# Gabrielcb/DaliID

Hardware: AMD Instinct MI355X
Metric: images/sec (train step) (higher is better)
Workload: dtype bf16; 1 GPU; configs[1]: ResNet-50 ReID bf16 256x128, PK batch 16x16=256 per GPU, center+proxy heads, Adam, EMA; global_batch=256, per_gpu_batch=256, parallelism=dp1

## Files before the change

### daliid_amd/csrc/conv.hip

```cpp
#include "gemm_tile.h"
#include "kernels.h"
#include <cstdlib>
#include <type_traits>
#include <vector>
#include <string>
#include <cstdio>

namespace dali {

__device__ __forceinline__ void decode_pixel(const GatherGeom& g, int p, int& n, int& ho, int& wo) {
    if (g.lhw >= 0 && g.lw >= 0) {
        n = p >> g.lhw;
        const int rem = p & ((1 << g.lhw) - 1);
        ho = rem >> g.lw;
        wo = rem & ((1 << g.lw) - 1);
    } else {
        const int hw = g.Hout * g.Wout;
        n = p / hw;
        const int rem = p - n * hw;
        ho = rem / g.Wout;
        wo = rem - ho * g.Wout;
    }
}

// ... 1295 lines not shown
                const bf16x8_t fb = *reinterpret_cast<const bf16x8_t*>(patch + (boff[j] ^ (uint32_t)(h << 5)));
#pragma unroll
                for (int i = 0; i < FM; ++i) acc[i][j] = __builtin_amdgcn_mfma_f32_16x16x32_bf16(fa[i], fb, acc[i][j], 0, 0, 0);
            }
        }
        asm volatile("s_waitcnt lgkmcnt(0)" ::: "memory");
        __builtin_amdgcn_s_barrier();
    }
    conv_epilogue_g<TM, TN, FM, FN, 4, NT, (EPI == 3 || EPI == 5) ? EPI : 2>(a, acc, 0, tn, smem, 0, wn);
}

}
#include "fused1x1.h"
namespace dali {

__device__ __forceinline__ int wg_swz(int row) { return (row & 3) | (((row >> 3) & 1) << 2); }

typedef short s16x4_t __attribute__((ext_vector_type(4)));

__device__ __forceinline__ bf16x8_t tr_frag(const uint16_t* tile, int chunk32, int lane) {
    const int g = lane >> 4, q = (lane & 15) >> 2, p = lane & 3;
    const int row0 = 8 * g + q, row1 = row0 + 4;
    const int off0 = row0 * 128 + ((chunk32 ^ wg_swz(row0)) << 4) + 4 * p;
    const int off1 = row1 * 128 + ((chunk32 ^ wg_swz(row1)) << 4) + 4 * p;
    typedef __attribute__((address_space(3))) s16x4_t* lds_ptr_t;
    const s16x4_t a = __builtin_amdgcn_ds_read_tr16_b64_v4i16((lds_ptr_t)(tile + off0));
    const s16x4_t b = __builtin_amdgcn_ds_read_tr16_b64_v4i16((lds_ptr_t)(tile + off1));
    typedef short s16x8_t __attribute__((ext_vector_type(8)));
    const s16x8_t v = {a[0], a[1], a[2], a[3], b[0], b[1], b[2], b[3]};
    return __builtin_bit_cast(bf16x8_t, v);
}

struct TrPair { s16x4_t lo, hi; };
__device__ __forceinline__ s16x4_t ds_read_tr_raw(const uint16_t* p) {
    typedef __attribute__((address_space(3))) const uint16_t* lds_cptr_t;
    const uint32_t addr = (uint32_t)(uintptr_t)(lds_cptr_t)p;
    s16x4_t v;
    asm volatile("ds_read_b64_tr_b16 %0, %1" : "=v"(v) : "v"(addr));
    return v;
}
__device__ __forceinline__ TrPair tr_frag_raw(const uint16_t* tile, int chunk32, int lane) {
    const int g = lane >> 4, q = (lane & 15) >> 2, p = lane & 3;
    const int row0 = 8 * g + q, row1 = row0 + 4;
    const int off0 = row0 * 128 + ((chunk32 ^ wg_swz(row0)) << 4) + 4 * p;
    const int off1 = row1 * 128 + ((chunk32 ^ wg_swz(row1)) << 4) + 4 * p;
    return TrPair{ds_read_tr_raw(tile + off0), ds_read_tr_raw(tile + off1)};
// ... 2 lines not shown
    typedef short s16x8_t __attribute__((ext_vector_type(8)));
    const s16x8_t v = {t.lo[0], t.lo[1], t.lo[2], t.lo[3], t.hi[0], t.hi[1], t.hi[2], t.hi[3]};
    return __builtin_bit_cast(bf16x8_t, v);
}
template <int N>
__device__ __forceinline__ void tr_settle(TrPair& a, TrPair& b, TrPair& c, TrPair& d) {
    static_assert(N == 0 || N == 8 || N == 10 || N == 16 || N == 18, "lgkmcnt immediates used by the callers");
    if constexpr (N == 0) asm volatile("s_waitcnt lgkmcnt(0)" : "+v"(a.lo), "+v"(a.hi), "+v"(b.lo), "+v"(b.hi), "+v"(c.lo), "+v"(c.hi), "+v"(d.lo), "+v"(d.hi));
    else if constexpr (N == 8) asm volatile("s_waitcnt lgkmcnt(8)" : "+v"(a.lo), "+v"(a.hi), "+v"(b.lo), "+v"(b.hi), "+v"(c.lo), "+v"(c.hi), "+v"(d.lo), "+v"(d.hi));
    else if constexpr (N == 10) asm volatile("s_waitcnt lgkmcnt(10)" : "+v"(a.lo), "+v"(a.hi), "+v"(b.lo), "+v"(b.hi), "+v"(c.lo), "+v"(c.hi), "+v"(d.lo), "+v"(d.hi));
    else if constexpr (N == 16) asm volatile("s_waitcnt lgkmcnt(15)" : "+v"(a.lo), "+v"(a.hi), "+v"(b.lo), "+v"(b.hi), "+v"(c.lo), "+v"(c.hi), "+v"(d.lo), "+v"(d.hi));
    else asm volatile("s_waitcnt lgkmcnt(15)" : "+v"(a.lo), "+v"(a.hi), "+v"(b.lo), "+v"(b.hi), "+v"(c.lo), "+v"(c.hi), "+v"(d.lo), "+v"(d.hi));
}

__device__ __forceinline__ void tr_settle_all(TrPair& a) { asm volatile("s_waitcnt lgkmcnt(0)" : "+v"(a.lo), "+v"(a.hi)); }

template <int FM, int FN>
__device__ __forceinline__ void store_slab_tiles(float* slab, const f32x4_t (&acc)[FM][FN], int m_first, int n_first, int Cm, int Ntot, int lane) {
    const int mr = m_first + (lane >> 4) * 4, nc = n_first + (lane & 15);
    if (m_first + 16 * FM <= Cm && n_first + 16 * FN <= Ntot) {
        float* row = slab + (size_t)mr * Ntot + nc;
#pragma unroll
        for (int i = 0; i < FM; ++i)
#pragma unroll
            for (int rr = 0; rr < 4; ++rr) {
                float* p = row + (size_t)(i * 16 + rr) * Ntot;
#pragma unroll
                for (int j = 0; j < FN; ++j) p[j * 16] = acc[i][j][rr];
            }
        return;
    }
#pragma unroll
    for (int i = 0; i < FM; ++i)
#pragma unroll
        for (int j = 0; j < FN; ++j) {
            const int n = nc + j * 16;
#pragma unroll
            for (int rr = 0; rr < 4; ++rr) {
                const int m = mr + i * 16 + rr;
                if (m < Cm && n < Ntot) slab[(size_t)m * Ntot + n] = acc[i][j][rr];
            }
        }
}

template <bool IN_BN>
__global__ __launch_bounds__(256) void igemm_wgrad_kernel(WGradArgs a, int tiles_m, int tiles_n) {
    constexpr int TILE = 32 * 128;
    __shared__ __attribute__((aligned(16))) uint16_t smem[2 * 2 * TILE];
    const int tid = threadIdx.x, lane = tid & 63, wave = tid >> 6;
    const int wm = wave >> 1, wn = wave & 1;
    const int tiles = tiles_m * tiles_n;
    const int tile = blockIdx.x % tiles, ks = blockIdx.x / tiles;
    const int tm = tile / tiles_n, tn = tile - tm * tiles_n;
    const int m0 = tm * 128, n0 = tn * 128;
    const GatherGeom g = a.g;

    const int c16 = tid & 15;
    const int am = m0 + c16 * 8;
// ... 1565 lines not shown
```

### daliid_amd/csrc/kernels.h

```cpp
#pragma once
#include "common.h"

namespace dali {

struct GatherGeom {
    int Hout, Wout;
    int Hin, Win;
    int Ck;
    int R, S, stride, pad;
    int mode;
    long long img_pitch;
    int row_pitch, pix_pitch;
    int lw, lhw;
    int sub, oph, opw, Hfull, Wfull;
    int r0, rstep, nr, s0, sstep, ns;
    int class_grid;
};

struct IGemmArgs {
    const uint16_t* W;
    const uint16_t* X;
    uint16_t* O;
    const uint16_t* Res;
    const uint8_t* res_mask;
// ... 31 lines not shown
    float* colsum;
};


struct TransposeJob { const uint16_t* w; uint16_t* wt; int Co, T, Ci, first_block; };
int launch_weight_transpose_batched(hipStream_t st, const TransposeJob* jobs, int n);

struct BnBwdSide { const uint16_t* raw; const float* mean; const float* invstd; const float* scale; const float* shift; };

int launch_igemm_conv(hipStream_t st, const IGemmArgs& a);
int gemm_profile_begin(hipStream_t st, int cls, double flops, const char* what);
void gemm_profile_end(hipStream_t st, int slot);
int igemm_conv_stat_tiles(int Cm, int P, int K);
bool conv_cat_act_supported(int Cm, int c1, int c2, int P, int parts = 1);
void wgrad_plan(int Cm, int Ntot, int P, int target_blocks, int* splits, int* pix_per_split, size_t* ws_bytes, int taps = 1, int halo_w = 0);
int launch_igemm_wgrad(hipStream_t st, const WGradArgs& a, float* out, int accumulate, float* colsum_out = nullptr, int colsum_rows = 0);
int launch_splitk_reduce2(hipStream_t st, const float* partial, float* out, size_t elems, int splits, int accumulate,
                          const float* partial2, float* out2, size_t elems2, int splits2);
bool wgrad_colsum_supported(int Cm, int Ntot, int taps, int P);
int launch_splitk_reduce(hipStream_t st, const float* partial, float* out, size_t elems, int splits, int accumulate);

int launch_linear_fwd(hipStream_t st, const uint16_t* x, const uint16_t* w, const float* bias, int act, const uint16_t* residual, uint16_t* y,
                      uint16_t* pre, const uint16_t* dact_pre, int rows, int K, int N, const float* row_scale = nullptr);
int launch_linear_wgrad(hipStream_t st, const uint16_t* x, const uint16_t* dy, float* dw, int rows, int K, int N, float* slab,
                        float* dbias = nullptr, float* cs_partial = nullptr, bool* bias_done = nullptr);
size_t linear_wgrad_colsum_floats(int rows, int K, int N);
int wgrad_colsum_rows(int Cm, int Ntot, int taps, int P, int splits);
size_t linear_wgrad_slab_bytes(int rows, int K, int N);

int launch_bnlin_stats(hipStream_t st, const uint16_t* W, const uint16_t* Wt, const float* gram, const float* m2, int C, int w, double count, const float* gamma,
// ... 6 lines not shown

constexpr int REDUCE_SMAX = 64;
inline size_t reduce_scratch_bytes(int C, int NV) { return (size_t)REDUCE_SMAX * C * NV * sizeof(double); }
int launch_bn_finalize(hipStream_t st, const float* partial, int tiles, int C, double count, const float* gamma, const float* beta,
                       float* rm, float* rv, float momentum, float eps, float* scale, float* shift, float* mean, float* invstd,
                       double* scratch);
int launch_bn_eval_coeffs(hipStream_t st, const float* gamma, const float* beta, const float* rm, const float* rv, float eps, int C,
                          float* scale, float* shift);
struct BnEvalJob { const float *gamma, *beta, *rm, *rv; float *scale, *shift; int C; };
struct BnEvalJobs { static constexpr int MAX = 56; BnEvalJob job[MAX]; };
int launch_bn_eval_coeffs_batched(hipStream_t st, const BnEvalJob* jobs, int n, float eps);
int launch_fold_cat_weights(hipStream_t st, const float* w3, const float* wd, const float* s3, const float* sd, const float* h3, const float* hd, int C, int w,
                            int cin, int parts, uint16_t* wcat, float* shcat);
int launch_bn_act(hipStream_t st, const uint16_t* raw, const float* scale, const float* shift, const uint16_t* idn, const uint16_t* raw2,
                  const float* scale2, const float* shift2, int relu, size_t elems, int C, uint16_t* y, uint8_t* mask_out);
int bn_bwd_blocks(int P, int C, int* rows_per_block);
size_t bn_bwd_partial_floats(int P, int C, bool dual);
int launch_bn_bwd(hipStream_t st, const uint16_t* g, const uint16_t* ymask, const uint8_t* ybits, const BnBwdSide& a, const BnBwdSide* b, int relu, int P, int C,
                  float* partial, float* coef_a, float* coef_b, float* dgamma_a, float* dbeta_a, float* dgamma_b, float* dbeta_b,
                  uint16_t* draw_a, uint16_t* draw_b, uint16_t* dz_out, double* scratch);
int launch_stem_pack_image(hipStream_t st, const float* img, int N, int H, int W, uint16_t* out);
int launch_stem_pack_weight(hipStream_t st, const float* w, int Cout, uint16_t* out);
bool stem_fused_supported(int N, int H, int W, int C);
bool stem_train_supported(int N, int H, int W, int C);
int stem_train_tiles(int N, int H);
int launch_stem_conv_stats(hipStream_t st, const uint16_t* ximg, const uint16_t* w_packed, int N, int H, int W, uint16_t* raw, float* stats);
int launch_stem_conv_bn_pool(hipStream_t st, const uint16_t* ximg, const uint16_t* w_packed, const float* scale, const float* shift, int N, int H, int W,
                             uint16_t* out);
int launch_stem_unpack_wgrad(hipStream_t st, const float* padded, int Cout, float* dw);
int launch_maxpool_bn_fwd(hipStream_t st, const uint16_t* raw, const float* scale, const float* shift, int N, int H, int W, int C,
// ... 35 lines not shown
```

### daliid_amd/csrc/nnops.hip

```cpp
#include "kernels.h"
#include "reduce_finish.h"

namespace dali {

__device__ __forceinline__ void unpack8(const uint4& v, float (&f)[8]) {
    f[0] = bf16_bits_to_f32(v.x & 0xffffu); f[1] = bf16_bits_to_f32(v.x >> 16);
    f[2] = bf16_bits_to_f32(v.y & 0xffffu); f[3] = bf16_bits_to_f32(v.y >> 16);
    f[4] = bf16_bits_to_f32(v.z & 0xffffu); f[5] = bf16_bits_to_f32(v.z >> 16);
    f[6] = bf16_bits_to_f32(v.w & 0xffffu); f[7] = bf16_bits_to_f32(v.w >> 16);
}
__device__ __forceinline__ uint4 pack8(const float (&f)[8]) {
    return make_uint4(pack_bf16x2(f[0], f[1]), pack_bf16x2(f[2], f[3]), pack_bf16x2(f[4], f[5]), pack_bf16x2(f[6], f[7]));
}
__device__ __forceinline__ void load8f(const float* __restrict__ p, float (&f)[8]) {
    const float4 a = *reinterpret_cast<const float4*>(p), b = *reinterpret_cast<const float4*>(p + 4);
    f[0] = a.x; f[1] = a.y; f[2] = a.z; f[3] = a.w; f[4] = b.x; f[5] = b.y; f[6] = b.z; f[7] = b.w;
}

struct FinBnFwd {
    double count;
    const float *gamma, *beta;
    float *running_mean, *running_var;
    float momentum, eps;
    float *scale, *shift, *mean_out, *invstd_out;
// ... 273 lines not shown
__global__ void stem_pack_weight_kernel(const float* __restrict__ w, int Cout, uint16_t* __restrict__ out) {
    const int i = blockIdx.x * blockDim.x + threadIdx.x;
    if (i >= Cout * 224) return;
    const int c = i & 3, s = (i >> 2) & 7, r = (i >> 5) % 7, o = i / 224;
    float v = 0.f;
    if (c < 3 && s < 7) v = w[((o * 7 + r) * 7 + s) * 3 + c];
    out[i] = f32_to_bf16_bits(v);
}
__global__ void stem_unpack_wgrad_kernel(const float* __restrict__ padded, int Cout, float* __restrict__ dw) {
    const int i = blockIdx.x * blockDim.x + threadIdx.x;
    if (i >= Cout * 147) return;
    const int c = i % 3, s = (i / 3) % 7, r = (i / 21) % 7, o = i / 147;
    dw[i] = padded[((o * 7 + r) * 8 + s) * 4 + c];
}

__global__ __launch_bounds__(256) void maxpool_bn_fwd_kernel(const uint16_t* __restrict__ raw, const float* __restrict__ scale,
                                                              const float* __restrict__ shift, int N, int H, int W, int C,
                                                              int Ho, int Wo, uint16_t* __restrict__ out, uint8_t* __restrict__ arg) {
    const int cpr = C >> 3;
    const size_t total = (size_t)N * Ho * Wo * cpr;
    for (size_t i = (size_t)blockIdx.x * 256 + threadIdx.x; i < total; i += (size_t)gridDim.x * 256) {
        const int cc = (int)(i % cpr) * 8;
        const size_t pix = i / cpr;
        const int wo = (int)(pix % Wo), ho = (int)((pix / Wo) % Ho), n = (int)(pix / ((size_t)Wo * Ho));
        float sc[8], sh[8], best[8];
        int bi[8];
        load8f(scale + cc, sc); load8f(shift + cc, sh);
#pragma unroll
        for (int t = 0; t < 8; ++t) { best[t] = -__builtin_inff(); bi[t] = 0; }
        uint4 q[9];
        bool ok[9];
#pragma unroll
        for (int r = 0; r < 3; ++r) {
            const int h = ho * 2 - 1 + r, hc = h < 0 ? 0 : (h >= H ? H - 1 : h);
#pragma unroll
            for (int s2 = 0; s2 < 3; ++s2) {
                const int w = wo * 2 - 1 + s2, wc = w < 0 ? 0 : (w >= W ? W - 1 : w);
                ok[r * 3 + s2] = h >= 0 && h < H && w >= 0 && w < W;
                q[r * 3 + s2] = *reinterpret_cast<const uint4*>(raw + (((size_t)n * H + hc) * W + wc) * C + cc);
            }
        }
#pragma unroll
        for (int k = 0; k < 9; ++k) {
            float v[8];
            unpack8(q[k], v);
#pragma unroll
            for (int t = 0; t < 8; ++t) {
                const float z = v[t] * sc[t] + sh[t];
                if (ok[k] && z > best[t]) { best[t] = z; bi[t] = k; }
            }
        }
        *reinterpret_cast<uint4*>(out + pix * C + cc) = pack8(best);
        uint32_t lo = 0, hi = 0;
#pragma unroll
        for (int t = 0; t < 4; ++t) { lo |= (uint32_t)bi[t] << (8 * t); hi |= (uint32_t)bi[t + 4] << (8 * t); }
        *reinterpret_cast<uint2*>(arg + pix * C + cc) = make_uint2(lo, hi);
    }
}

__device__ __forceinline__ void maxpool_gather_dz(const uint16_t* __restrict__ dp, const uint8_t* __restrict__ arg, int n, int h, int w,
                                                  int cc, int C, int Ho, int Wo, float (&dz)[8]) {
    const int ho0 = h >> 1, wo0 = w >> 1;
    const int rh[2] = {1 + (h & 1), 0}, rw[2] = {1 + (w & 1), 0};
    const bool vh[2] = {ho0 < Ho, (h & 1) && ho0 + 1 < Ho}, vw[2] = {wo0 < Wo, (w & 1) && wo0 + 1 < Wo};
    uint4 gq[4];
    uint2 aq[4];
#pragma unroll
    for (int k = 0; k < 4; ++k) {
        const int a = k >> 1, b = k & 1;
        const int ho = min(ho0 + a, Ho - 1), wo = min(wo0 + b, Wo - 1);
        const size_t o = (((size_t)n * Ho + ho) * Wo + wo) * C + cc;
        aq[k] = *reinterpret_cast<const uint2*>(arg + o);
// ... 437 lines not shown
    return DALI_OK;
}
int launch_fold_cat_weights(hipStream_t st, const float* w3, const float* wd, const float* s3, const float* sd, const float* h3, const float* hd, int C, int w,
                            int cin, int parts, uint16_t* wcat, float* shcat) {
    const size_t n = (size_t)C * parts * (w + cin);
    hipLaunchKernelGGL(fold_cat_weights_kernel, dim3(grid_for(n, 1024)), dim3(256), 0, st, w3, wd, s3, sd, h3, hd, C, w, cin, parts, wcat, shcat);
    DALI_LAUNCH_CHECK();
    return DALI_OK;
}
int launch_bn_act(hipStream_t st, const uint16_t* raw, const float* scale, const float* shift, const uint16_t* idn, const uint16_t* raw2,
                  const float* scale2, const float* shift2, int relu, size_t elems, int C, uint16_t* y, uint8_t* mask_out) {
    const size_t chunks = elems / 8;
    hipLaunchKernelGGL(bn_act_kernel, dim3(grid_for(chunks)), dim3(256), 0, st, raw, scale, shift, idn, raw2, scale2, shift2, relu, chunks, C, y, mask_out);
    DALI_LAUNCH_CHECK();
    return DALI_OK;
}
int bn_bwd_blocks(int P, int C, int* rows_per_block) {
    const int rif = 256 / (C / 8);
    int blocks = (P + rif * 8 - 1) / (rif * 8);
    if (blocks > 1024) blocks = 1024;
    if (blocks < 1) blocks = 1;
    int rpb = (P + blocks - 1) / blocks;
    rpb = (rpb + rif - 1) / rif * rif;
    blocks = (P + rpb - 1) / rpb;
    *rows_per_block = rpb;
    return blocks;
}
int launch_bn_bwd(hipStream_t st, const uint16_t* g, const uint16_t* ymask, const uint8_t* ybits, const BnBwdSide& a, const BnBwdSide* b, int relu, int P, int C,
                  float* partial, float* coef_a, float* coef_b, float* dgamma_a, float* dbeta_a, float* dgamma_b, float* dbeta_b,
                  uint16_t* draw_a, uint16_t* draw_b, uint16_t* dz_out, double* scratch) {
// ... 183 lines not shown
    float* coef_b = reinterpret_cast<float*>(ws + align_up(pf * 4, 256) + align_up((size_t)C * 12, 256));
    double* scratch = reinterpret_cast<double*>(ws + align_up(pf * 4, 256) + 2 * align_up((size_t)C * 12, 256));
    BnBwdSide a{raw_a, mean_a, invstd_a, scale_a, shift_a};
    BnBwdSide b{raw_b, mean_b, invstd_b, scale_b, nullptr};
    return launch_bn_bwd((hipStream_t)stream, g, ymask, ybits, a, dual ? &b : nullptr, relu, (int)pixels, C, partial, coef_a, coef_b, dgamma_a, dbeta_a,
                         dgamma_b, dbeta_b, draw_a, draw_b, dz_out, scratch);
}

extern "C" int dali_maxpool_bn_fwd(dali_ctx* ctx, void* stream, const uint16_t* raw, const float* scale, const float* shift, int n, int h,
                                   int w, int C, uint16_t* out, uint8_t* arg) {
    DALI_REQUIRE(ctx && raw && scale && shift && out && arg, "dali_maxpool_bn_fwd: null argument");
    DALI_REQUIRE(C % 8 == 0 && n > 0 && h > 0 && w > 0, "dali_maxpool_bn_fwd: bad shape");
    return launch_maxpool_bn_fwd((hipStream_t)stream, raw, scale, shift, n, h, w, C, out, arg);
}

extern "C" int dali_maxpool_bn_bwd(dali_ctx* ctx, void* stream, const uint16_t* dpool, const uint8_t* arg, const uint16_t* raw,
                                   const float* mean, const float* invstd, const float* scale, int n, int h, int w, int C,
                                   float* dgamma, float* dbeta, uint16_t* draw) {
    DALI_REQUIRE(ctx && dpool && arg && raw && mean && invstd && scale && dgamma && dbeta && draw, "dali_maxpool_bn_bwd: null argument");
    DALI_REQUIRE(C % 8 == 0 && C <= 2048, "dali_maxpool_bn_bwd: C must be a multiple of 8, <= 2048");
    const size_t pf = bn_bwd_partial_floats(n * h * w, C, false);
    const size_t need = align_up(pf * 4, 256) + align_up((size_t)C * 12, 256) + reduce_scratch_bytes(C, 2);
    char* ws = static_cast<char*>(workspace(ctx, need));
    if (!ws) return DALI_ERR_NOMEM;
    return launch_maxpool_bn_bwd((hipStream_t)stream, dpool, arg, raw, mean, invstd, scale, n, h, w, C, reinterpret_cast<float*>(ws),
                                 reinterpret_cast<float*>(ws + align_up(pf * 4, 256)), dgamma, dbeta, draw,
                                 reinterpret_cast<double*>(ws + align_up(pf * 4, 256) + align_up((size_t)C * 12, 256)));
}

extern "C" int dali_head_pool_fwd(dali_ctx* ctx, void* stream, const uint16_t* x, int n, int hw, int C, int mode, float* f, int16_t* arg) {
// ... 24 lines not shown
```

### daliid_amd/csrc/resnet_plan.hip

```cpp
#include "kernels.h"
#include <cstdio>
#include <cstring>
#include <new>
#include <string>
#include <vector>

using namespace dali;

namespace {

struct TensorInfo { std::string name; int64_t offset, numel; int shape[4]; int ndim; };

struct Conv {
    int cin, cout, r, s, stride, pad, hin, win, hout, wout;
    int64_t w_off;
    uint16_t* w_bf16;
    uint16_t* wt_bf16;
};
struct Bn {
    int C;
    int64_t g_off, b_off;
    int64_t rm_off, rv_off;
    float *scale, *shift, *mean, *invstd, *coef;
};
// ... 389 lines not shown
}

extern "C" int dali_resnet_forward(dali_resnet* net, void* stream, const float* images, int training, float* emb) {
    DALI_REQUIRE(net && net->P && images && emb, "dali_resnet_forward: null argument or net not bound");
    hipStream_t st = (hipStream_t)stream;
    const bool tr = training != 0;
    net->fwd_training = tr;
    int rc;
    if (!tr) {
        std::vector<BnEvalJob> jobs;
        auto add = [&](Bn& b) { jobs.push_back(BnEvalJob{net->P + b.g_off, net->P + b.b_off, net->B + b.rm_off, net->B + b.rv_off, b.scale, b.shift, b.C}); };
        add(net->stem_bn);
        for (auto& b : net->blocks) { add(b.b1); add(b.b2); add(b.b3); if (b.has_ds) add(b.bd); }
        if ((rc = launch_bn_eval_coeffs_batched(st, jobs.data(), (int)jobs.size(), 1e-5f))) return rc;
    }
    if ((rc = launch_stem_pack_image(st, images, net->N, net->H, net->W, net->ximg))) return rc;
    if (!tr && stem_fused_supported(net->N, net->H, net->W, net->stem.cout)) {
        if ((rc = launch_stem_conv_bn_pool(st, net->ximg, net->w_stem, net->stem_bn.scale, net->stem_bn.shift, net->N, net->H, net->W, net->pool0))) return rc;
    } else {
    if (tr && stem_train_supported(net->N, net->H, net->W, net->stem.cout)) {
        if ((rc = launch_stem_conv_stats(st, net->ximg, net->w_stem, net->N, net->H, net->W, net->raw0, net->stat_partial))) return rc;
        if ((rc = bn_train(net, st, net->stem_bn, stem_train_tiles(net->N, net->H), (double)net->N * net->stem_h * net->stem_w))) return rc;
    } else {
        IGemmArgs a{};
        a.W = net->w_stem; a.X = net->ximg; a.O = net->raw0; a.Res = nullptr; a.in_scale = nullptr; a.in_shift = nullptr; a.in_relu = 0;
        a.stats = tr ? net->stat_partial : nullptr;
        a.Cm = net->stem.cout; a.P = net->N * net->stem_h * net->stem_w;
        a.g = stem_geom(net);
        if ((rc = launch_igemm_conv(st, a))) return rc;
        if (tr && (rc = bn_train(net, st, net->stem_bn, igemm_conv_stat_tiles(a.Cm, a.P, 224), (double)a.P))) return rc;
    }
    if ((rc = launch_maxpool_bn_fwd(st, net->raw0, net->stem_bn.scale, net->stem_bn.shift, net->N, net->stem_h, net->stem_w, net->stem.cout,
                                    net->pool0, net->pool_arg))) return rc;
    }
    const uint16_t* x = net->pool0;
    for (auto& b : net->blocks) {
        b.x = const_cast<uint16_t*>(x);
        const size_t e1 = (size_t)net->N * b.hin * b.win * b.width, e2 = (size_t)net->N * b.hout * b.wout * b.width;
        if (!tr) {
            if ((rc = conv_bn_relu_eval(net, st, b.c1, b.b1, x, b.a1))) return rc;
            if ((rc = conv_bn_relu_eval(net, st, b.c2, b.b2, b.a1, b.a2))) return rc;
        } else {
            if ((rc = conv_bn_fwd(net, st, b.c1, b.b1, x, nullptr, b.raw1, tr))) return rc;
            if ((rc = launch_bn_act(st, b.raw1, b.b1.scale, b.b1.shift, nullptr, nullptr, nullptr, nullptr, 1, e1, b.width, b.a1, nullptr))) return rc;
            if ((rc = conv_bn_fwd(net, st, b.c2, b.b2, b.a1, nullptr, b.raw2, tr))) return rc;
            if ((rc = launch_bn_act(st, b.raw2, b.b2.scale, b.b2.shift, nullptr, nullptr, nullptr, nullptr, 1, e2, b.width, b.a2, nullptr))) return rc;
        }
        const int Pout = net->N * b.hout * b.wout;
        if (tr) {
            const Conv sq = square_conv(b.c3);
            WGradArgs wa{};
            wa.dY = b.a2; wa.X = b.a2; wa.partial = net->wgrad_slab; wa.Cm = b.width; wa.P = Pout; wa.Ntot = b.width;
            wa.g = conv_geom(sq, 0);
            size_t wsb;
            wgrad_plan(wa.Cm, wa.Ntot, wa.P, 512, &wa.splits, &wa.pix_per_split, &wsb, 1, 0);
            const bool fused_cs = wgrad_colsum_supported(wa.Cm, wa.Ntot, 1, wa.P);
            if (fused_cs) wa.colsum = net->cs_partial;
            if ((rc = launch_igemm_wgrad(st, wa, b.gram, 0, fused_cs ? b.m2 : nullptr, fused_cs ? wgrad_colsum_rows(wa.Cm, wa.Ntot, 1, wa.P, wa.splits) : 0))) return rc;
            if (!fused_cs && (rc = launch_colsum(st, b.a2, Pout, b.width, b.m2, net->cs_partial, net->red_scratch))) return rc;
            if ((rc = launch_bnlin_stats(st, b.c3.w_bf16, b.c3.wt_bf16, b.gram, b.m2, b.cout, b.width, (double)Pout, net->P + b.b3.g_off, net->P + b.b3.b_off,
                                         net->B + b.b3.rm_off, net->B + b.b3.rv_off, 0.1f, 1e-5f, b.ut, b.dot, b.b3.scale, b.b3.shift, b.b3.mean,
                                         b.b3.invstd))) return rc;
        }
        if (!tr && b.cat_eval) {
            if ((rc = launch_fold_cat_weights(st, net->P + b.c3.w_off, net->P + b.cd.w_off, b.b3.scale, b.bd.scale, b.b3.shift, b.bd.shift, b.cout, b.width,
                                              b.cin, 2, b.wcat, b.shcat))) return rc;
            IGemmArgs ca{};
            ca.W = b.wcat; ca.X = b.a2; ca.X2 = x; ca.Ck1 = b.width; ca.x_rep = 2; ca.O = b.y; ca.out_shift = b.shcat; ca.out_relu = 1;
            ca.Cm = b.cout; ca.P = Pout;
            Conv cat = b.c3;
            cat.cin = 2 * (b.width + b.cin);
            ca.g = conv_geom(cat, 0);
            if ((rc = launch_igemm_conv(st, ca))) return rc;
            x = b.y;
            continue;
        }
        IGemmArgs a{};
        a.W = b.c3.w_bf16; a.X = b.a2; a.O = b.y; a.Res = x; a.out_scale = b.b3.scale; a.out_shift = b.b3.shift; a.out_relu = 1;
        if (b.has_ds) {
            if ((rc = conv_bn_fwd(net, st, b.cd, b.bd, x, nullptr, b.rawd, tr))) return rc;
            a.Res = b.rawd; a.res_scale = b.bd.scale; a.bias = b.bd.shift;
            if (b.lin_ds && tr) {
                Conv sq = b.cd;
                sq.cout = b.cd.cin;
                WGradArgs wa{};
                wa.dY = x; wa.X = x; wa.partial = net->wgrad_slab; wa.Cm = b.cin; wa.P = Pout; wa.Ntot = b.cin;
                wa.g = conv_geom(sq, 0);
                size_t wsb;
                wgrad_plan(wa.Cm, wa.Ntot, wa.P, 512, &wa.splits, &wa.pix_per_split, &wsb, 1, 0);
                const bool fused_cs = wgrad_colsum_supported(wa.Cm, wa.Ntot, 1, wa.P);
                if (fused_cs) wa.colsum = net->cs_partial;
                if ((rc = launch_igemm_wgrad(st, wa, b.gram_d, 0, fused_cs ? b.m2_d : nullptr, fused_cs ? wgrad_colsum_rows(wa.Cm, wa.Ntot, 1, wa.P, wa.splits) : 0))) return rc;
                if (!fused_cs && (rc = launch_colsum(st, x, Pout, b.cin, b.m2_d, net->cs_partial, net->red_scratch))) return rc;
                if ((rc = launch_bnlin_ut(st, b.cd.w_bf16, b.gram_d, b.cout, b.cin, b.ut_d))) return rc;
            }
        }
        a.bits_out = tr ? b.ybits : nullptr;
        a.Cm = b.cout; a.P = Pout; a.g = conv_geom(b.c3, 0);
        if ((rc = launch_igemm_conv(st, a))) return rc;
        x = b.y;
    }
    if ((rc = launch_head_pool_fwd(st, x, net->N, net->head_hw, net->feat_dim, net->feature_mode, net->feat, net->head_arg))) return rc;
    return launch_bn1d_fwd(st, net->feat, net->N, net->feat_dim, net->P + net->neck.g_off, net->P + net->neck.b_off, net->B + net->neck.rm_off,
                           net->B + net->neck.rv_off, tr ? 1 : 0, 0.1f, 1e-5f, emb, net->neck_mean, net->neck_invstd);
}

static int block_backward(dali_resnet* net, hipStream_t st, Block& b, const uint8_t* prev_bits) {
    int rc;
    uint16_t* dz = net->cur_dy;
    const int Pout = net->N * b.hout * b.wout, Pin = net->N * b.hin * b.win;
// ... 174 lines not shown
```

### include/daliid_debug.h

```cpp
#ifndef DALIID_DEBUG_H
#define DALIID_DEBUG_H

#ifdef __cplusplus
extern "C" {
#endif

int dali_debug_reload_env(void);

int dali_debug_set_conv_stamps(void* dev_ptr);

int dali_debug_wgrad_splits(int Cm, int Ntot, int P, int taps, int halo_w);

int dali_debug_splitk_reduce(void* stream, const float* partial, float* out, long long elems, int splits, int accumulate);

struct dali_resnet;
int dali_debug_resnet_backward_block(struct dali_resnet* net, void* stream, const float* d_emb, int block);

#ifdef __cplusplus
}
#endif
#endif
```

Measured before the change: 17400 images/s.

## Fuse BN-activation and maxpool with Gram/colsum computation for linearized BN stats

Adds two fused kernels. One applies BN+ReLU to the conv2 output while also computing the activation's Gram matrix and column sums via MFMA. The other does the stem maxpool+BN and the Gram matrix for the first downsample block. These replace the separate bn_act pass plus a re-read of the activation by the wgrad Gram kernel, saving a full activation read and a kernel launch per block. The cost is more complex kernels whose occupancy and split planning may differ from the tuned wgrad path. The fused path falls back when shapes are not covered.

```diff
diff --git a/daliid_amd/csrc/conv.hip b/daliid_amd/csrc/conv.hip
--- a/daliid_amd/csrc/conv.hip
+++ b/daliid_amd/csrc/conv.hip
@@ -1,5 +1,6 @@
 #include "gemm_tile.h"
 #include "kernels.h"
+#include "wgrad_frag.h"
 #include <cstdlib>
 #include <type_traits>
 #include <vector>
@@ -1333,22 +1334,6 @@
 #include "fused1x1.h"
 namespace dali {
 
-__device__ __forceinline__ int wg_swz(int row) { return (row & 3) | (((row >> 3) & 1) << 2); }
-
-typedef short s16x4_t __attribute__((ext_vector_type(4)));
-
-__device__ __forceinline__ bf16x8_t tr_frag(const uint16_t* tile, int chunk32, int lane) {
-    const int g = lane >> 4, q = (lane & 15) >> 2, p = lane & 3;
-    const int row0 = 8 * g + q, row1 = row0 + 4;
-    const int off0 = row0 * 128 + ((chunk32 ^ wg_swz(row0)) << 4) + 4 * p;
-    const int off1 = row1 * 128 + ((chunk32 ^ wg_swz(row1)) << 4) + 4 * p;
-    typedef __attribute__((address_space(3))) s16x4_t* lds_ptr_t;
-    const s16x4_t a = __builtin_amdgcn_ds_read_tr16_b64_v4i16((lds_ptr_t)(tile + off0));
-    const s16x4_t b = __builtin_amdgcn_ds_read_tr16_b64_v4i16((lds_ptr_t)(tile + off1));
-    typedef short s16x8_t __attribute__((ext_vector_type(8)));
-    const s16x8_t v = {a[0], a[1], a[2], a[3], b[0], b[1], b[2], b[3]};
-    return __builtin_bit_cast(bf16x8_t, v);
-}
 
 struct TrPair { s16x4_t lo, hi; };
 __device__ __forceinline__ s16x4_t ds_read_tr_raw(const uint16_t* p) {
@@ -1381,34 +1366,6 @@
 }
 
 __device__ __forceinline__ void tr_settle_all(TrPair& a) { asm volatile("s_waitcnt lgkmcnt(0)" : "+v"(a.lo), "+v"(a.hi)); }
-
-template <int FM, int FN>
-__device__ __forceinline__ void store_slab_tiles(float* slab, const f32x4_t (&acc)[FM][FN], int m_first, int n_first, int Cm, int Ntot, int lane) {
-    const int mr = m_first + (lane >> 4) * 4, nc = n_first + (lane & 15);
-    if (m_first + 16 * FM <= Cm && n_first + 16 * FN <= Ntot) {
-        float* row = slab + (size_t)mr * Ntot + nc;
-#pragma unroll
-        for (int i = 0; i < FM; ++i)
-#pragma unroll
-            for (int rr = 0; rr < 4; ++rr) {
-                float* p = row + (size_t)(i * 16 + rr) * Ntot;
-#pragma unroll
-                for (int j = 0; j < FN; ++j) p[j * 16] = acc[i][j][rr];
-            }
-        return;
-    }
-#pragma unroll
-    for (int i = 0; i < FM; ++i)
-#pragma unroll
-        for (int j = 0; j < FN; ++j) {
-            const int n = nc + j * 16;
-#pragma unroll
-            for (int rr = 0; rr < 4; ++rr) {
-                const int m = mr + i * 16 + rr;
-                if (m < Cm && n < Ntot) slab[(size_t)m * Ntot + n] = acc[i][j][rr];
-            }
-        }
-}
 
 template <bool IN_BN>
 __global__ __launch_bounds__(256) void igemm_wgrad_kernel(WGradArgs a, int tiles_m, int tiles_n) {
diff --git a/daliid_amd/csrc/kernels.h b/daliid_amd/csrc/kernels.h
--- a/daliid_amd/csrc/kernels.h
+++ b/daliid_amd/csrc/kernels.h
@@ -69,6 +69,7 @@
 int igemm_conv_stat_tiles(int Cm, int P, int K);
 bool conv_cat_act_supported(int Cm, int c1, int c2, int P, int parts = 1);
 void wgrad_plan(int Cm, int Ntot, int P, int target_blocks, int* splits, int* pix_per_split, size_t* ws_bytes, int taps = 1, int halo_w = 0);
+int wgrad_pick_cfg(int Cm, int Ntot, int taps, int P, int halo_w);
 int launch_igemm_wgrad(hipStream_t st, const WGradArgs& a, float* out, int accumulate, float* colsum_out = nullptr, int colsum_rows = 0);
 int launch_splitk_reduce2(hipStream_t st, const float* partial, float* out, size_t elems, int splits, int accumulate,
                           const float* partial2, float* out2, size_t elems2, int splits2);
@@ -105,6 +106,12 @@
                             int cin, int parts, uint16_t* wcat, float* shcat);
 int launch_bn_act(hipStream_t st, const uint16_t* raw, const float* scale, const float* shift, const uint16_t* idn, const uint16_t* raw2,
                   const float* scale2, const float* shift2, int relu, size_t elems, int C, uint16_t* y, uint8_t* mask_out);
+bool bn_act_gram_supported(int P, int w);
+int launch_bn_act_gram(hipStream_t st, const uint16_t* raw, const float* scale, const float* shift, int P, int w, uint16_t* y, float* slab,
+                       float* cs_slab, float* gram, float* m2);
+bool maxpool_bn_gram_supported(int N, int H, int W, int C);
+int launch_maxpool_bn_gram(hipStream_t st, const uint16_t* raw, const float* scale, const float* shift, int N, int H, int W, int C, uint16_t* out,
+                           uint8_t* arg, float* slab, float* cs_slab, float* gram, float* m2);
 int bn_bwd_blocks(int P, int C, int* rows_per_block);
 size_t bn_bwd_partial_floats(int P, int C, bool dual);
 int launch_bn_bwd(hipStream_t st, const uint16_t* g, const uint16_t* ymask, const uint8_t* ybits, const BnBwdSide& a, const BnBwdSide* b, int relu, int P, int C,
diff --git a/daliid_amd/csrc/nnops.hip b/daliid_amd/csrc/nnops.hip
--- a/daliid_amd/csrc/nnops.hip
+++ b/daliid_amd/csrc/nnops.hip
@@ -1,5 +1,7 @@
 #include "kernels.h"
 #include "reduce_finish.h"
+#include "wgrad_frag.h"
+#include <cstdio>
 
 namespace dali {
 
@@ -311,6 +313,29 @@
     dw[i] = padded[((o * 7 + r) * 8 + s) * 4 + c];
 }
 
+__device__ __forceinline__ void maxpool_bn_taps(const uint4 (&q)[9], const bool (&ok)[9], const float (&sc)[8], const float (&sh)[8], uint4& out,
+                                                uint2& arg) {
+    float best[8];
+    int bi[8];
+#pragma unroll
+    for (int t = 0; t < 8; ++t) { best[t] = -__builtin_inff(); bi[t] = 0; }
+#pragma unroll
+    for (int k = 0; k < 9; ++k) {
+        float v[8];
+        unpack8(q[k], v);
+#pragma unroll
+        for (int t = 0; t < 8; ++t) {
+            const float z = v[t] * sc[t] + sh[t];
+            if (ok[k] && z > best[t]) { best[t] = z; bi[t] = k; }
+        }
+    }
+    out = pack8(best);
+    uint32_t lo = 0, hi = 0;
+#pragma unroll
+    for (int t = 0; t < 4; ++t) { lo |= (uint32_t)bi[t] << (8 * t); hi |= (uint32_t)bi[t + 4] << (8 * t); }
+    arg = make_uint2(lo, hi);
+}
+
 __global__ __launch_bounds__(256) void maxpool_bn_fwd_kernel(const uint16_t* __restrict__ raw, const float* __restrict__ scale,
                                                               const float* __restrict__ shift, int N, int H, int W, int C,
                                                               int Ho, int Wo, uint16_t* __restrict__ out, uint8_t* __restrict__ arg) {
@@ -320,11 +345,8 @@
         const int cc = (int)(i % cpr) * 8;
         const size_t pix = i / cpr;
         const int wo = (int)(pix % Wo), ho = (int)((pix / Wo) % Ho), n = (int)(pix / ((size_t)Wo * Ho));
-        float sc[8], sh[8], best[8];
-        int bi[8];
+        float sc[8], sh[8];
         load8f(scale + cc, sc); load8f(shift + cc, sh);
-#pragma unroll
-        for (int t = 0; t < 8; ++t) { best[t] = -__builtin_inff(); bi[t] = 0; }
         uint4 q[9];
         bool ok[9];
 #pragma unroll
@@ -337,22 +359,192 @@
                 q[r * 3 + s2] = *reinterpret_cast<const uint4*>(raw + (((size_t)n * H + hc) * W + wc) * C + cc);
             }
         }
-#pragma unroll
-        for (int k = 0; k < 9; ++k) {
-            float v[8];
-            unpack8(q[k], v);
-#pragma unroll
-            for (int t = 0; t < 8; ++t) {
-                const float z = v[t] * sc[t] + sh[t];
-                if (ok[k] && z > best[t]) { best[t] = z; bi[t] = k; }
+        uint4 o;
+        uint2 oa;
+        maxpool_bn_taps(q, ok, sc, sh, o, oa);
+        *reinterpret_cast<uint4*>(out + pix * C + cc) = o;
+        *reinterpret_cast<uint2*>(arg + pix * C + cc) = oa;
+    }
+}
+
+struct BnGramArgs {
+    const uint16_t* raw;
+    const float *scale, *shift;
+    uint16_t* out;
+    uint8_t* arg;
+    float *partial, *colsum;
+    int pps;
+    int H, Ho;
+};
+
+template <int W>
+struct GramTiles {
+    static constexpr int FM = W == 64 ? 1 : 4, FN = 4;
+    int mf0, nf0;
+    bool do_cs;
+    f32x4_t acc[FM][FN], cs[FM];
+    __device__ explicit GramTiles(int wave) {
+        mf0 = W == 64 ? wave : (wave >> 1) * 4;
+        nf0 = W == 64 ? 0 : (wave & 1) * 4;
+        do_cs = W == 64 || (wave & 1) == 0;
+#pragma unroll
+        for (int i = 0; i < FM; ++i) {
+            cs[i] = f32x4_t{0.f, 0.f, 0.f, 0.f};
+#pragma unroll
+            for (int j = 0; j < FN; ++j) acc[i][j] = f32x4_t{0.f, 0.f, 0.f, 0.f};
+        }
+    }
+    __device__ void step(const uint16_t* img, int lane) {
+        typedef short ones_vec_t __attribute__((ext_vector_type(8)));
+        const bf16x8_t ones = __builtin_bit_cast(bf16x8_t, ones_vec_t{0x3F80, 0x3F80, 0x3F80, 0x3F80, 0x3F80, 0x3F80, 0x3F80, 0x3F80});
+        bf16x8_t fa[FM];
+#pragma unroll
+        for (int i = 0; i < FM; ++i) fa[i] = tr_frag(img, mf0 + i, lane);
+#pragma unroll
+        for (int j = 0; j < FN; ++j) {
+            const bf16x8_t fb = tr_frag(img, nf0 + j, lane);
+#pragma unroll
+            for (int i = 0; i < FM; ++i) acc[i][j] = __builtin_amdgcn_mfma_f32_16x16x32_bf16(fa[i], fb, acc[i][j], 0, 0, 0);
+        }
+        if (do_cs) {
+#pragma unroll
+            for (int i = 0; i < FM; ++i) cs[i] = __builtin_amdgcn_mfma_f32_16x16x32_bf16(fa[i], ones, cs[i], 0, 0, 0);
+        }
+    }
+    __device__ void store(const BnGramArgs& a, int ks, int lane) const {
+        store_slab_tiles<FM, FN>(a.partial + (size_t)ks * W * W, acc, 16 * mf0, 16 * nf0, W, W, lane);
+        if (do_cs && (lane & 15) == 0) {
+#pragma unroll
+            for (int i = 0; i < FM; ++i)
+#pragma unroll
+                for (int rr = 0; rr < 4; ++rr) a.colsum[(size_t)ks * W + 16 * (mf0 + i) + (lane >> 4) * 4 + rr] = cs[i][rr];
+        }
+    }
+};
+
+template <int W, int U>
+__global__ __launch_bounds__(256, 2) void bn_act_gram_kernel(BnGramArgs a) {
+    static_assert(W == 64 || W == 128, "widths of the plan");
+    constexpr int CPR = W / 8, RSTEP = 256 / CPR;
+    constexpr int CPT = CPR / 8;
+    constexpr int NB = U * CPT;
+    __shared__ __attribute__((aligned(16))) uint16_t smem[U * 32 * 128];
+    const int tid = threadIdx.x, lane = tid & 63;
+    const int wave = __builtin_amdgcn_readfirstlane(tid >> 6);
+    const int ks = blockIdx.x;
+    const int c16 = tid % CPR, row0 = tid / CPR;
+    float sc[8], sh[8];
+    load8f(a.scale + c16 * 8, sc); load8f(a.shift + c16 * 8, sh);
+    auto load = [&](int ph, uint4 (&q)[NB]) {
+#pragma unroll
+        for (int u = 0; u < U; ++u)
+#pragma unroll
+            for (int c = 0; c < CPT; ++c) {
+                const size_t pix = (size_t)ks * a.pps + (ph * U + u) * 32 + row0 + c * RSTEP;
+                q[u * CPT + c] = *reinterpret_cast<const uint4*>(a.raw + pix * W + c16 * 8);
             }
-        }
-        *reinterpret_cast<uint4*>(out + pix * C + cc) = pack8(best);
-        uint32_t lo = 0, hi = 0;
-#pragma unroll
-        for (int t = 0; t < 4; ++t) { lo |= (uint32_t)bi[t] << (8 * t); hi |= (uint32_t)bi[t + 4] << (8 * t); }
-        *reinterpret_cast<uint2*>(arg + pix * C + cc) = make_uint2(lo, hi);
-    }
+    };
+    GramTiles<W> gt(wave);
+    const int nph = a.pps / (32 * U);
+    uint4 cur[NB], nxt[NB];
+    load(0, cur);
+    for (int ph = 0; ph < nph; ++ph) {
+        if (ph + 1 < nph) load(ph + 1, nxt);
+#pragma unroll
+        for (int u = 0; u < U; ++u)
+#pragma unroll
+            for (int c = 0; c < CPT; ++c) {
+                const int row = row0 + c * RSTEP;
+                const size_t pix = (size_t)ks * a.pps + (ph * U + u) * 32 + row;
+                float v[8];
+                unpack8(cur[u * CPT + c], v);
+#pragma unroll
+                for (int t = 0; t < 8; ++t) v[t] = v[t] * sc[t] + sh[t];
+#pragma unroll
+                for (int t = 0; t < 8; ++t) v[t] = fmaxf(v[t], 0.f);
+                const uint4 o = pack8(v);
+                *reinterpret_cast<uint4*>(a.out + pix * W + c16 * 8) = o;
+                *reinterpret_cast<uint4*>(smem + u * 32 * 128 + wg_img_off(row, c16)) = o;
+            }
+        __syncthreads();
+#pragma unroll
+        for (int u = 0; u < U; ++u) gt.step(smem + u * 32 * 128, lane);
+        __syncthreads();
+#pragma unroll
+        for (int i = 0; i < NB; ++i) cur[i] = nxt[i];
+    }
+    gt.store(a, ks, lane);
+}
+
+typedef uint32_t u32x4_t __attribute__((ext_vector_type(4)));
+template <int U>
+__global__ __launch_bounds__(256, 2) void maxpool_bn_gram_kernel(BnGramArgs a) {
+    constexpr int C = 64, WIN = 64, WO = 32, ROWS = 2 * U + 1, RB = WIN * C;
+    constexpr int NB = ROWS * 2;
+    __shared__ __attribute__((aligned(16))) uint16_t stage[ROWS * RB];
+    __shared__ __attribute__((aligned(16))) uint16_t smem[U * 32 * 128];
+    const int tid = threadIdx.x, lane = tid & 63;
+    const int wave = __builtin_amdgcn_readfirstlane(tid >> 6);
+    const int ks = blockIdx.x;
+    const int c16 = tid & 7, wo = tid >> 3;
+    float sc[8], sh[8];
+    load8f(a.scale + c16 * 8, sc); load8f(a.shift + c16 * 8, sh);
+    auto rows_of = [&](int ph, int& n, int& ho0) __attribute__((always_inline)) {
+        const int t = (ks * a.pps) / WO + ph * U;
+        n = t / a.Ho; ho0 = t - n * a.Ho;
+    };
+    auto load = [&](int ph, u32x4_t (&q)[NB]) __attribute__((always_inline)) {
+        int n, ho0;
+        rows_of(ph, n, ho0);
+#pragma unroll
+        for (int j = 0; j < ROWS; ++j) {
+            const int h = 2 * ho0 - 1 + j, hc = h < 0 ? 0 : (h >= a.H ? a.H - 1 : h);
+#pragma unroll
+            for (int c = 0; c < 2; ++c)
+                q[j * 2 + c] = *reinterpret_cast<const u32x4_t*>(a.raw + ((size_t)n * a.H + hc) * RB + (tid + 256 * c) * 8);
+        }
+    };
+    GramTiles<C> gt(wave);
+    const int nph = a.pps / (32 * U);
+    u32x4_t rg[NB];
+    load(0, rg);
+    for (int ph = 0; ph < nph; ++ph) {
+#pragma unroll
+        for (int j = 0; j < ROWS; ++j)
+#pragma unroll
+            for (int c = 0; c < 2; ++c) *reinterpret_cast<u32x4_t*>(stage + j * RB + (tid + 256 * c) * 8) = rg[j * 2 + c];
+        __syncthreads();
+        if (ph + 1 < nph) load(ph + 1, rg);
+        int n, ho0;
+        rows_of(ph, n, ho0);
+#pragma unroll
+        for (int u = 0; u < U; ++u) {
+            const int ho = ho0 + u;
+            uint4 q[9];
+            bool ok[9];
+#pragma unroll
+            for (int r = 0; r < 3; ++r) {
+                const int h = ho * 2 - 1 + r;
+#pragma unroll
+                for (int s2 = 0; s2 < 3; ++s2) {
+                    const int w = wo * 2 - 1 + s2, wc = w < 0 ? 0 : (w >= WIN ? WIN - 1 : w);
+                    ok[r * 3 + s2] = h >= 0 && h < a.H && w >= 0 && w < WIN;
+                    q[r * 3 + s2] = *reinterpret_cast<const uint4*>(stage + (2 * u + r) * RB + wc * C + c16 * 8);
+                }
+            }
+            uint4 o;
+            uint2 oa;
+            maxpool_bn_taps(q, ok, sc, sh, o, oa);
+            const size_t pix = ((size_t)n * a.Ho + ho) * WO + wo;
+            *reinterpret_cast<uint4*>(a.out + pix * C + c16 * 8) = o;
+            *reinterpret_cast<uint2*>(a.arg + pix * C + c16 * 8) = oa;
+            *reinterpret_cast<uint4*>(smem + u * 32 * 128 + wg_img_off(wo, c16)) = o;
+        }
+        __syncthreads();
+#pragma unroll
+        for (int u = 0; u < U; ++u) gt.step(smem + u * 32 * 128, lane);
+    }
+    gt.store(a, ks, lane);
 }
 
 __device__ __forceinline__ void maxpool_gather_dz(const uint16_t* __restrict__ dp, const uint8_t* __restrict__ arg, int n, int h, int w,
@@ -820,6 +1012,51 @@
     hipLaunchKernelGGL(bn_act_kernel, dim3(grid_for(chunks)), dim3(256), 0, st, raw, scale, shift, idn, raw2, scale2, shift2, relu, chunks, C, y, mask_out);
     DALI_LAUNCH_CHECK();
     return DALI_OK;
+}
+
+constexpr int BNG_U64 = 8, BNG_U128 = 4, BNG_U_POOL = 2;
+static int bn_gram_splits(int P, int w, int u, int* pps) {
+    if (!(w == 64 || w == 128) || P <= 0 || wgrad_pick_cfg(w, w, 1, P, 0) != 0 || !wgrad_colsum_supported(w, w, 1, P)) return 0;
+    int sp = 0;
+    size_t wsb = 0;
+    wgrad_plan(w, w, P, 512, &sp, pps, &wsb, 1, 0);
+    return ((long long)sp * *pps == P && *pps % (32 * u) == 0) ? sp : 0;
+}
+bool bn_act_gram_supported(int P, int w) { int pps; return bn_gram_splits(P, w, w == 64 ? BNG_U64 : BNG_U128, &pps) > 0; }
+bool maxpool_bn_gram_supported(int N, int H, int W, int C) {
+    const int Ho = (H + 2 - 3) / 2 + 1;
+    int pps;
+    return C == 64 && W == 64 && H >= 2 && Ho % BNG_U_POOL == 0 && (long long)N * H * W * C < (1ll << 31) &&
+           bn_gram_splits(N * Ho * 32, C, BNG_U_POOL, &pps) > 0;
+}
+static int launch_bn_gram(hipStream_t st, BnGramArgs a, int P, int w, bool pool, float* gram, float* m2) {
+    int pps;
+    const int sp = bn_gram_splits(P, w, pool ? BNG_U_POOL : (w == 64 ? BNG_U64 : BNG_U128), &pps);
+    if (!sp) { set_error("bn_gram: shape not covered (P=%d w=%d)", P, w); return DALI_ERR_INVALID; }
+    a.pps = pps;
+    char what[96] = "";
+    snprintf(what, sizeof what, "bngram,Cm=%d,K=%d,P=%d,pool=%d", w, w, P, pool ? 1 : 0);
+    const int slot = gemm_profile_begin(st, 1, 2.0 * w * w * (double)P, what);
+    if (pool) hipLaunchKernelGGL(maxpool_bn_gram_kernel<BNG_U_POOL>, dim3(sp), dim3(256), 0, st, a);
+    else if (w == 64) hipLaunchKernelGGL((bn_act_gram_kernel<64, BNG_U64>), dim3(sp), dim3(256), 0, st, a);
+    else hipLaunchKernelGGL((bn_act_gram_kernel<128, BNG_U128>), dim3(sp), dim3(256), 0, st, a);
+    gemm_profile_end(st, slot);
+    DALI_LAUNCH_CHECK();
+    return launch_splitk_reduce2(st, a.partial, gram, (size_t)w * w, sp, 0, a.colsum, m2, (size_t)w, wgrad_colsum_rows(w, w, 1, P, sp));
+}
+int launch_bn_act_gram(hipStream_t st, const uint16_t* raw, const float* scale, const float* shift, int P, int w, uint16_t* y, float* slab,
+                       float* cs_slab, float* gram, float* m2) {
+    BnGramArgs a{};
+    a.raw = raw; a.scale = scale; a.shift = shift; a.out = y; a.partial = slab; a.colsum = cs_slab;
+    return launch_bn_gram(st, a, P, w, false, gram, m2);
+}
+int launch_maxpool_bn_gram(hipStream_t st, const uint16_t* raw, const float* scale, const float* shift, int N, int H, int W, int C, uint16_t* out,
+                           uint8_t* arg, float* slab, float* cs_slab, float* gram, float* m2) {
+    if (!maxpool_bn_gram_supported(N, H, W, C)) { set_error("maxpool_bn_gram: shape not covered"); return DALI_ERR_INVALID; }
+    BnGramArgs a{};
+    a.raw = raw; a.scale = scale; a.shift = shift; a.out = out; a.arg = arg; a.partial = slab; a.colsum = cs_slab;
+    a.H = H; a.Ho = (H + 2 - 3) / 2 + 1;
+    return launch_bn_gram(st, a, N * a.Ho * 32, C, true, gram, m2);
 }
 int bn_bwd_blocks(int P, int C, int* rows_per_block) {
     const int rif = 256 / (C / 8);
@@ -1033,6 +1270,19 @@
     return launch_maxpool_bn_fwd((hipStream_t)stream, raw, scale, shift, n, h, w, C, out, arg);
 }
 
+extern "C" int dali_debug_bn_act_gram(void* stream, const uint16_t* raw, const float* scale, const float* shift, int P, int w, uint16_t* a,
+                                      float* slab, float* cs_slab, float* gram, float* m2) {
+    DALI_REQUIRE(raw && scale && shift && a && slab && cs_slab && gram && m2, "dali_debug_bn_act_gram: null argument");
+    DALI_REQUIRE(bn_act_gram_supported(P, w), "dali_debug_bn_act_gram: shape not covered (P=%d w=%d)", P, w);
+    return launch_bn_act_gram((hipStream_t)stream, raw, scale, shift, P, w, a, slab, cs_slab, gram, m2);
+}
+extern "C" int dali_debug_maxpool_bn_gram(void* stream, const uint16_t* raw, const float* scale, const float* shift, int n, int h, int w, int C,
+                                          uint16_t* out, uint8_t* arg, float* slab, float* cs_slab, float* gram, float* m2) {
+    DALI_REQUIRE(raw && scale && shift && out && arg && slab && cs_slab && gram && m2, "dali_debug_maxpool_bn_gram: null argument");
+    DALI_REQUIRE(maxpool_bn_gram_supported(n, h, w, C), "dali_debug_maxpool_bn_gram: shape not covered");
+    return launch_maxpool_bn_gram((hipStream_t)stream, raw, scale, shift, n, h, w, C, out, arg, slab, cs_slab, gram, m2);
+}
+
 extern "C" int dali_maxpool_bn_bwd(dali_ctx* ctx, void* stream, const uint16_t* dpool, const uint8_t* arg, const uint16_t* raw,
                                    const float* mean, const float* invstd, const float* scale, int n, int h, int w, int C,
                                    float* dgamma, float* dbeta, uint16_t* draw) {
diff --git a/daliid_amd/csrc/resnet_plan.hip b/daliid_amd/csrc/resnet_plan.hip
--- a/daliid_amd/csrc/resnet_plan.hip
+++ b/daliid_amd/csrc/resnet_plan.hip
@@ -427,6 +427,8 @@
         for (auto& b : net->blocks) { add(b.b1); add(b.b2); add(b.b3); if (b.has_ds) add(b.bd); }
         if ((rc = launch_bn_eval_coeffs_batched(st, jobs.data(), (int)jobs.size(), 1e-5f))) return rc;
     }
+    const bool pool_gram = tr && !net->blocks.empty() && net->blocks[0].lin_ds && net->blocks[0].cin == net->stem.cout &&
+                           maxpool_bn_gram_supported(net->N, net->stem_h, net->stem_w, net->stem.cout);
     if ((rc = launch_stem_pack_image(st, images, net->N, net->H, net->W, net->ximg))) return rc;
     if (!tr && stem_fused_supported(net->N, net->H, net->W, net->stem.cout)) {
         if ((rc = launch_stem_conv_bn_pool(st, net->ximg, net->w_stem, net->stem_bn.scale, net->stem_bn.shift, net->N, net->H, net->W, net->pool0))) return rc;
@@ -443,8 +445,12 @@
         if ((rc = launch_igemm_conv(st, a))) return rc;
         if (tr && (rc = bn_train(net, st, net->stem_bn, igemm_conv_stat_tiles(a.Cm, a.P, 224), (double)a.P))) return rc;
     }
-    if ((rc = launch_maxpool_bn_fwd(st, net->raw0, net->stem_bn.scale, net->stem_bn.shift, net->N, net->stem_h, net->stem_w, net->stem.cout,
-                                    net->pool0, net->pool_arg))) return rc;
+    if (pool_gram) {
+        Block& b0 = net->blocks[0];
+        if ((rc = launch_maxpool_bn_gram(st, net->raw0, net->stem_bn.scale, net->stem_bn.shift, net->N, net->stem_h, net->stem_w, net->stem.cout,
+                                         net->pool0, net->pool_arg, net->wgrad_slab, net->cs_partial, b0.gram_d, b0.m2_d))) return rc;
+    } else if ((rc = launch_maxpool_bn_fwd(st, net->raw0, net->stem_bn.scale, net->stem_bn.shift, net->N, net->stem_h, net->stem_w, net->stem.cout,
+                                           net->pool0, net->pool_arg))) return rc;
     }
     const uint16_t* x = net->pool0;
     for (auto& b : net->blocks) {
@@ -457,20 +463,27 @@
             if ((rc = conv_bn_fwd(net, st, b.c1, b.b1, x, nullptr, b.raw1, tr))) return rc;
             if ((rc = launch_bn_act(st, b.raw1, b.b1.scale, b.b1.shift, nullptr, nullptr, nullptr, nullptr, 1, e1, b.width, b.a1, nullptr))) return rc;
             if ((rc = conv_bn_fwd(net, st, b.c2, b.b2, b.a1, nullptr, b.raw2, tr))) return rc;
-            if ((rc = launch_bn_act(st, b.raw2, b.b2.scale, b.b2.shift, nullptr, nullptr, nullptr, nullptr, 1, e2, b.width, b.a2, nullptr))) return rc;
         }
         const int Pout = net->N * b.hout * b.wout;
+        const bool a2_gram = tr && bn_act_gram_supported(Pout, b.width);
+        if (a2_gram) {
+            if ((rc = launch_bn_act_gram(st, b.raw2, b.b2.scale, b.b2.shift, Pout, b.width, b.a2, net->wgrad_slab, net->cs_partial, b.gram, b.m2))) return rc;
+        } else if (tr && (rc = launch_bn_act(st, b.raw2, b.b2.scale, b.b2.shift, nullptr, nullptr, nullptr, nullptr, 1, e2, b.width, b.a2, nullptr))) {
+            return rc;
+        }
         if (tr) {
-            const Conv sq = square_conv(b.c3);
-            WGradArgs wa{};
-            wa.dY = b.a2; wa.X = b.a2; wa.partial = net->wgrad_slab; wa.Cm = b.width; wa.P = Pout; wa.Ntot = b.width;
-            wa.g = conv_geom(sq, 0);
-            size_t wsb;
-            wgrad_plan(wa.Cm, wa.Ntot, wa.P, 512, &wa.splits, &wa.pix_per_split, &wsb, 1, 0);
-            const bool fused_cs = wgrad_colsum_supported(wa.Cm, wa.Ntot, 1, wa.P);
-            if (fused_cs) wa.colsum = net->cs_partial;
-            if ((rc = launch_igemm_wgrad(st, wa, b.gram, 0, fused_cs ? b.m2 : nullptr, fused_cs ? wgrad_colsum_rows(wa.Cm, wa.Ntot, 1, wa.P, wa.splits) : 0))) return rc;
-            if (!fused_cs && (rc = launch_colsum(st, b.a2, Pout, b.width, b.m2, net->cs_partial, net->red_scratch))) return rc;
+            if (!a2_gram) {
+                const Conv sq = square_conv(b.c3);
+                WGradArgs wa{};
+                wa.dY = b.a2; wa.X = b.a2; wa.partial = net->wgrad_slab; wa.Cm = b.width; wa.P = Pout; wa.Ntot = b.width;
+                wa.g = conv_geom(sq, 0);
+                size_t wsb;
+                wgrad_plan(wa.Cm, wa.Ntot, wa.P, 512, &wa.splits, &wa.pix_per_split, &wsb, 1, 0);
+                const bool fused_cs = wgrad_colsum_supported(wa.Cm, wa.Ntot, 1, wa.P);
+                if (fused_cs) wa.colsum = net->cs_partial;
+                if ((rc = launch_igemm_wgrad(st, wa, b.gram, 0, fused_cs ? b.m2 : nullptr, fused_cs ? wgrad_colsum_rows(wa.Cm, wa.Ntot, 1, wa.P, wa.splits) : 0))) return rc;
+                if (!fused_cs && (rc = launch_colsum(st, b.a2, Pout, b.width, b.m2, net->cs_partial, net->red_scratch))) return rc;
+            }
             if ((rc = launch_bnlin_stats(st, b.c3.w_bf16, b.c3.wt_bf16, b.gram, b.m2, b.cout, b.width, (double)Pout, net->P + b.b3.g_off, net->P + b.b3.b_off,
                                          net->B + b.b3.rm_off, net->B + b.b3.rv_off, 0.1f, 1e-5f, b.ut, b.dot, b.b3.scale, b.b3.shift, b.b3.mean,
                                          b.b3.invstd))) return rc;
@@ -493,7 +506,7 @@
         if (b.has_ds) {
             if ((rc = conv_bn_fwd(net, st, b.cd, b.bd, x, nullptr, b.rawd, tr))) return rc;
             a.Res = b.rawd; a.res_scale = b.bd.scale; a.bias = b.bd.shift;
-            if (b.lin_ds && tr) {
+            if (b.lin_ds && tr && !(pool_gram && x == net->pool0)) {
                 Conv sq = b.cd;
                 sq.cout = b.cd.cin;
                 WGradArgs wa{};
@@ -505,8 +518,8 @@
                 if (fused_cs) wa.colsum = net->cs_partial;
                 if ((rc = launch_igemm_wgrad(st, wa, b.gram_d, 0, fused_cs ? b.m2_d : nullptr, fused_cs ? wgrad_colsum_rows(wa.Cm, wa.Ntot, 1, wa.P, wa.splits) : 0))) return rc;
                 if (!fused_cs && (rc = launch_colsum(st, x, Pout, b.cin, b.m2_d, net->cs_partial, net->red_scratch))) return rc;
-                if ((rc = launch_bnlin_ut(st, b.cd.w_bf16, b.gram_d, b.cout, b.cin, b.ut_d))) return rc;
             }
+            if (b.lin_ds && tr && (rc = launch_bnlin_ut(st, b.cd.w_bf16, b.gram_d, b.cout, b.cin, b.ut_d))) return rc;
         }
         a.bits_out = tr ? b.ybits : nullptr;
         a.Cm = b.cout; a.P = Pout; a.g = conv_geom(b.c3, 0);
diff --git a/daliid_amd/csrc/wgrad_frag.h b/daliid_amd/csrc/wgrad_frag.h
--- /dev/null
+++ b/daliid_amd/csrc/wgrad_frag.h
@@ -0,0 +1,53 @@
+#pragma once
+#include "common.h"
+
+namespace dali {
+
+__device__ __forceinline__ int wg_swz(int row) { return (row & 3) | (((row >> 3) & 1) << 2); }
+
+__device__ __forceinline__ int wg_img_off(int row, int c16) { return row * 128 + (((c16 >> 1) ^ wg_swz(row)) << 4) + (c16 & 1) * 8; }
+
+typedef short s16x4_t __attribute__((ext_vector_type(4)));
+
+__device__ __forceinline__ bf16x8_t tr_frag(const uint16_t* tile, int chunk32, int lane) {
+    const int g = lane >> 4, q = (lane & 15) >> 2, p = lane & 3;
+    const int row0 = 8 * g + q, row1 = row0 + 4;
+    const int off0 = row0 * 128 + ((chunk32 ^ wg_swz(row0)) << 4) + 4 * p;
+    const int off1 = row1 * 128 + ((chunk32 ^ wg_swz(row1)) << 4) + 4 * p;
+    typedef __attribute__((address_space(3))) s16x4_t* lds_ptr_t;
+    const s16x4_t a = __builtin_amdgcn_ds_read_tr16_b64_v4i16((lds_ptr_t)(tile + off0));
+    const s16x4_t b = __builtin_amdgcn_ds_read_tr16_b64_v4i16((lds_ptr_t)(tile + off1));
+    typedef short s16x8_t __attribute__((ext_vector_type(8)));
+    const s16x8_t v = {a[0], a[1], a[2], a[3], b[0], b[1], b[2], b[3]};
+    return __builtin_bit_cast(bf16x8_t, v);
+}
+
+template <int FM, int FN>
+__device__ __forceinline__ void store_slab_tiles(float* slab, const f32x4_t (&acc)[FM][FN], int m_first, int n_first, int Cm, int Ntot, int lane) {
+    const int mr = m_first + (lane >> 4) * 4, nc = n_first + (lane & 15);
+    if (m_first + 16 * FM <= Cm && n_first + 16 * FN <= Ntot) {
+        float* row = slab + (size_t)mr * Ntot + nc;
+#pragma unroll
+        for (int i = 0; i < FM; ++i)
+#pragma unroll
+            for (int rr = 0; rr < 4; ++rr) {
+                float* p = row + (size_t)(i * 16 + rr) * Ntot;
+#pragma unroll
+                for (int j = 0; j < FN; ++j) p[j * 16] = acc[i][j][rr];
+            }
+        return;
+    }
+#pragma unroll
+    for (int i = 0; i < FM; ++i)
+#pragma unroll
+        for (int j = 0; j < FN; ++j) {
+            const int n = nc + j * 16;
+#pragma unroll
+            for (int rr = 0; rr < 4; ++rr) {
+                const int m = mr + i * 16 + rr;
+                if (m < Cm && n < Ntot) slab[(size_t)m * Ntot + n] = acc[i][j][rr];
+            }
+        }
+}
+
+}
diff --git a/include/daliid_debug.h b/include/daliid_debug.h
--- a/include/daliid_debug.h
+++ b/include/daliid_debug.h
@@ -1,5 +1,6 @@
 #ifndef DALIID_DEBUG_H
 #define DALIID_DEBUG_H
+#include <stdint.h>
 
 #ifdef __cplusplus
 extern "C" {
@@ -13,6 +14,11 @@
 
 int dali_debug_splitk_reduce(void* stream, const float* partial, float* out, long long elems, int splits, int accumulate);
 
+int dali_debug_bn_act_gram(void* stream, const uint16_t* raw, const float* scale, const float* shift, int P, int w, uint16_t* a,
+                           float* slab, float* cs_slab, float* gram, float* m2);
+int dali_debug_maxpool_bn_gram(void* stream, const uint16_t* raw, const float* scale, const float* shift, int n, int h, int w, int C,
+                               uint16_t* out, uint8_t* arg, float* slab, float* cs_slab, float* gram, float* m2);
+
 struct dali_resnet;
 int dali_debug_resnet_backward_block(struct dali_resnet* net, void* stream, const float* d_emb, int block);
 
```

Measured after the change: 17510 images/s (median of 6 runs). Within noise of the previous version (+0.7%).
